# ebu/libear

Measured on AMD Instinct MI355X. Metric: Msamples/s, higher is better.
Workload: dtype f32 io / f16x2-split MFMA, f32 accumulate

## Files before the change

### libear_amd/csrc/api_core.hip

```cpp
#include <cctype>
#include <cerrno>
#include <cmath>
#include <cstdlib>
#include <string>
#include <memory>
#include <mutex>
#include <type_traits>

#include "common.h"
#include "curves.h"
#include "gain_kernels.h"
#include "gain_mfma.h"
#include "gain_h2.h"
#include "gain_h2_t1.h"
#include "gain_p2.h"
#include "gain_hg.h"
#include "gain_f32g.h"

namespace earhip {

static_assert(kSplitTile == 256, "MixLaunch::tile() and tiles_aligned(256, ...) assume the 4-wave tile");

static thread_local std::string g_last_error;
void set_last_error(const std::string &msg) { g_last_error = msg; }
// ... 363 lines not shown
    case GainKernel::Grid: launch_grid(c); break;
    case GainKernel::Pieces: launch_pieces(c); break;
    case GainKernel::Hinge:
      launch_hinge(c);
      if (c.standby) launch_pieces(c);
      break;
  }
  if (ev) EARHIP_HIP(hipEventRecord(ev[3], ctx->stream));
  EARHIP_HIP(hipGetLastError());
  MixResult res;
  res.gated = kind == GainKernel::Hinge && c.w.gate;
  res.device_form = c.w.wide_cur != nullptr;
  res.hinge_robust = res.gated && c.hg_robust;
  res.grew = c.w.grew;
  return res;
}

size_t hinge_build_allow_lds(const hipDeviceProp_t &prop) {
  const size_t want = 128 * 1024, dflt = 64 * 1024;
  const size_t device_max = std::max((size_t)prop.sharedMemPerBlock, (size_t)prop.maxSharedMemoryPerMultiProcessor);
  size_t ask = std::min(want, device_max > 4096 ? device_max - 4096 : dflt);
  if (ask <= dflt) return dflt;
  bool ok = true;
  for_each_hinge_build([&](auto T, auto NW) {
    ok = ok && hipFuncSetAttribute(reinterpret_cast<const void *>(&k_hinge_build<decltype(T)::value, decltype(NW)::value>),
                                   hipFuncAttributeMaxDynamicSharedMemorySize, (int)ask) == hipSuccess;
  });
  if (!ok) (void)hipGetLastError();
  return ok ? ask : dflt;
}

struct GainStage {
  earhip_ctx *ctx;
  int n_in, n_out;
  CurveSet curves;
  DevBuf<SegDesc> desc;
  DevBuf<float> parts;
  std::vector<float> rows;
  bool force_ramp;
  GainStage(earhip_ctx *c, int ni, int no, bool ramp = false)
      : ctx(c), n_in(ni), n_out(no), curves(ni, no, 1, ramp), force_ramp(ramp) {}

  void run_device(int64_t t_call, int nsamples, const float *in_dev, size_t in_stride,
                  float *out_dev, size_t out_stride) {
    curves.commit(ctx);
    const bool strict = ctx->strict || n_in == 1 || force_ramp;
    const MixLaunch ml = plan_mix(ctx, curves.plan(), n_in, nsamples, strict, 32, curves.stats(t_call, in_stride, (size_t)nsamples, false));
    if (ml.kind == GainKernel::Hinge) curves.ensure_kinks(ctx);
    desc.reserve(scratch_units(curves, ml, n_in));
    const size_t row_stride = ((size_t)nsamples + 3) & ~(size_t)3;
    if (ml.gsplit > 1) parts.reserve(row_stride * n_out * ml.gsplit);
    launch_gain_mix_summed(ctx, curves, ml, strict, t_call, nsamples, in_dev, in_stride, out_dev, out_stride, parts.p, row_stride, desc.p,
                           nullptr, nullptr);
  }

  void run_host(int64_t t_call, const float *const *in, float *const *out, int64_t r0,
                int64_t r1) {
    const int n = (int)(r1 - r0);
    if (n <= 0) return;
    const size_t stride = ((size_t)n + 3) & ~(size_t)3;
    ctx->pin_in.reserve(stride * n_in);
    ctx->pin_out.reserve(stride * n_out);
    ctx->dev_in.reserve(stride * n_in);
    ctx->dev_out.reserve(stride * n_out);
    for (int c = 0; c < n_in; c++)
      std::memcpy(ctx->pin_in.p + c * stride, in[c] + r0, sizeof(float) * n);
    EARHIP_HIP(hipMemcpyAsync(ctx->dev_in.p, ctx->pin_in.p, sizeof(float) * stride * n_in,
                              hipMemcpyHostToDevice, ctx->stream));
    run_device(t_call, n, ctx->dev_in.p, stride, ctx->dev_out.p, stride);
    EARHIP_HIP(hipMemcpyAsync(ctx->pin_out.p, ctx->dev_out.p, sizeof(float) * stride * n_out,
                              hipMemcpyDeviceToHost, ctx->stream));
    EARHIP_HIP(hipStreamSynchronize(ctx->stream));
    for (int c = 0; c < n_out; c++)
      std::memcpy(out[c] + r0, ctx->pin_out.p + c * stride, sizeof(float) * n);
  }
};

}

using namespace earhip;

static const char *const kOptNames[OPT_COUNT] = {
    "SPL", "MFMA", "XSCALE", "WAVES", "TPW", "NRT", "H2_TILE", "H2_WGS", "H2_RUNS", "P2_TILE", "P2_PAIRS", "P2_WGS", "HINGE", "HG_TILE", "HBUILD_TPW",
    "BUILD_TPW", "K2_WG", "K2_OWN_BLOCK", "RUN", "GSPLIT", "PROBE_RUNS", "BLOCK_GROUPS", "DEBUG_TIMING", "TAILCUT", "HOST_CHUNK_MB", "HOST_THREADS", "HG_ROBUST", "BUILD_2K", "HOST_BIND", "HOST_NT", "HOST_FIRST", "H2_PAIR"};

static int parse_option_value(const std::string &key, const char *text) {
  char *end = nullptr;
  errno = 0;
  const long v = std::strtol(text, &end, 10);
  while (end && *end && std::isspace((unsigned char)*end)) end++;
  if (end == text || (end && *end) || errno == ERANGE || v < -(1L << 30) || v > (1L << 30))
    fail_invalid("option '" + key + "': '" + std::string(text) + "' is not an integer");
  return (int)v;
}

void earhip_ctx::apply_options() {
  spl = 4, use_mfma = 3, x_scale_log2 = 14, x_scale_auto = true, max_waves = 4, tiles_per_wg = 4, tiles_per_wg_forced = false, nrt = 8;
  if (has(OPT_SPL) && (get(OPT_SPL) == 2 || get(OPT_SPL) == 4)) spl = get(OPT_SPL);
  if (has(OPT_MFMA)) use_mfma = get(OPT_MFMA);
  if (has(OPT_XSCALE) && get(OPT_XSCALE) >= -64 && get(OPT_XSCALE) <= 64)
    x_scale_log2 = get(OPT_XSCALE), x_scale_auto = false;
  if (has(OPT_WAVES) && get(OPT_WAVES) >= 1 && get(OPT_WAVES) <= 8) max_waves = get(OPT_WAVES);
  if (has(OPT_TPW) && get(OPT_TPW) >= 1 && get(OPT_TPW) <= 8) tiles_per_wg = get(OPT_TPW), tiles_per_wg_forced = true;
  if (has(OPT_NRT) && (get(OPT_NRT) == 4 || get(OPT_NRT) == 8)) nrt = get(OPT_NRT);
}

struct earhip_gain_interp {
  std::unique_ptr<GainStage> stage;
};

struct PolicyCache {
  std::vector<std::unique_ptr<GainStage>> stages;
  GainStage *get(earhip_ctx *ctx, int n_in, int n_out, bool ramp) {
    for (auto &s : stages)
      if (s->n_in == n_in && s->n_out == n_out && s->force_ramp == ramp) return s.get();
    stages.emplace_back(new GainStage(ctx, n_in, n_out, ramp));
    return stages.back().get();
  }
};
static std::vector<std::pair<earhip_ctx *, std::unique_ptr<PolicyCache>>> g_policy;
static std::mutex g_policy_mutex;
static PolicyCache *policy_cache(earhip_ctx *ctx) {
  std::lock_guard<std::mutex> lock(g_policy_mutex);
  for (auto &p : g_policy)
    if (p.first == ctx) return p.second.get();
  g_policy.emplace_back(ctx, std::unique_ptr<PolicyCache>(new PolicyCache));
  return g_policy.back().second.get();
}

static __global__ void k_clock_probe(unsigned long long *out) {
  out[0] = clock64();
  out[1] = wall_clock64();
}

static __global__ void __launch_bounds__(256) k_read_linear(const f32x4 *in, float *out, size_t n4) {
  f32x4 acc = {0.0f, 0.0f, 0.0f, 0.0f};
  size_t i = (size_t)blockIdx.x * 256 + threadIdx.x;
  const size_t step = (size_t)gridDim.x * 256;
  for (; i + 3 * step < n4; i += 4 * step) {
    const f32x4 a = __builtin_nontemporal_load(in + i), b = __builtin_nontemporal_load(in + i + step);
    const f32x4 c = __builtin_nontemporal_load(in + i + 2 * step), d = __builtin_nontemporal_load(in + i + 3 * step);
    acc += (a + b) + (c + d);
  }
  for (; i < n4; i += step) acc += __builtin_nontemporal_load(in + i);
  if (acc[0] + acc[1] + acc[2] + acc[3] == 123.456f) out[0] = 1.0f;
}
static __global__ void __launch_bounds__(256) k_read_rows(const float *in, float *out, int rows, size_t stride) {
  constexpr int DEPTH = 4;
  const int lane = threadIdx.x & 63, w = threadIdx.x >> 6, li = lane & 15, kg = lane >> 4;
  const float *base = in + (size_t)blockIdx.x * 256 + w * 64 + li * 4;
  auto row = [&](int r) { return base + (size_t)min(r, rows - 1) * stride; };
  f32x4 acc = {0.0f, 0.0f, 0.0f, 0.0f};
  f32x4 ring[DEPTH][8];
#pragma unroll
  for (int d = 0; d < DEPTH; d++)
#pragma unroll
    for (int q = 0; q < 8; q++)
      ring[d][q] = __builtin_nontemporal_load((const f32x4 *)row(d * 32 + kg * 8 + q));
  for (int r0 = 0; r0 < rows; r0 += 32 * DEPTH) {
#pragma unroll
    for (int d = 0; d < DEPTH; d++) {
#pragma unroll
      for (int q = 0; q < 8; q++) acc += ring[d][q];
      const int rn = r0 + 32 * DEPTH + d * 32;
      if (rn < rows)
#pragma unroll
        for (int q = 0; q < 8; q++)
// ... 406 lines not shown
```

### libear_amd/csrc/common.h

```cpp
#pragma once

#include <hip/hip_runtime.h>

#include <cstdint>
#include <cstdio>
#include <string>
#include <vector>

#include "../../include/earhip.h"

namespace earhip {

struct Error {
  int code;
  std::string msg;
};

void set_last_error(const std::string &msg);

template <typename F>
int guarded(F &&f) {
  try {
    f();
    return EARHIP_OK;
// ... 15 lines not shown
[[noreturn]] inline void fail_internal(const std::string &m) {
  throw Error{EARHIP_INTERNAL_ERROR, "internal error: " + m};
}
inline void require(bool ok, const char *m) {
  if (!ok) fail_invalid(m);
}

#define EARHIP_HIP(expr)                                                        \
  do {                                                                          \
    hipError_t e_ = (expr);                                                     \
    if (e_ != hipSuccess)                                                       \
      throw ::earhip::Error{EARHIP_DEVICE_ERROR,                                \
                            std::string("internal error: HIP: ") +              \
                                hipGetErrorString(e_) + " in " #expr};          \
  } while (0)

inline bool is_pow2(size_t v) { return v && !(v & (v - 1)); }

template <typename T>
struct DevBuf {
  T *p = nullptr;
  size_t n = 0;
  DevBuf() = default;
  DevBuf(const DevBuf &) = delete;
  DevBuf &operator=(const DevBuf &) = delete;
  ~DevBuf() { release(); }
  void release() {
    if (p) (void)hipFree(p);
    p = nullptr;
    n = 0;
  }
  void alloc(size_t count) {
    release();
    if (count == 0) count = 1;
    EARHIP_HIP(hipMalloc((void **)&p, count * sizeof(T)));
    n = count;
  }
  void alloc_zero(size_t count, hipStream_t s) {
    alloc(count);
    EARHIP_HIP(hipMemsetAsync(p, 0, n * sizeof(T), s));
  }
  void reserve(size_t count) {
    if (count > n) alloc(count);
  }
  void upload(const std::vector<T> &v) {
    alloc(v.size());
    if (!v.empty()) EARHIP_HIP(hipMemcpy(p, v.data(), sizeof(T) * v.size(), hipMemcpyHostToDevice));
  }
};

template <typename T>
struct PinBuf {
  T *p = nullptr;
  size_t n = 0;
  PinBuf() = default;
  PinBuf(const PinBuf &) = delete;
  PinBuf &operator=(const PinBuf &) = delete;
  ~PinBuf() {
    if (p) (void)hipHostFree(p);
  }
  void reserve(size_t count) {
    if (count <= n) return;
    if (p) (void)hipHostFree(p);
    p = nullptr;
    n = 0;
    EARHIP_HIP(hipHostMalloc((void **)&p, count * sizeof(T), hipHostMallocDefault));
    n = count;
  }
};

}

struct earhip_vbs;
namespace earhip {
void vbs_orphan(earhip_vbs *v);
}

namespace earhip {
enum Opt {
  OPT_SPL, OPT_MFMA, OPT_XSCALE, OPT_WAVES, OPT_TPW, OPT_NRT,
  OPT_H2_TILE, OPT_H2_WGS, OPT_H2_RUNS, OPT_P2_TILE, OPT_P2_PAIRS, OPT_P2_WGS, OPT_HINGE, OPT_HG_TILE, OPT_HBUILD_TPW, OPT_BUILD_TPW,
  OPT_K2_WG, OPT_K2_OWN_BLOCK, OPT_RUN, OPT_GSPLIT,
  OPT_PROBE_RUNS, OPT_BLOCK_GROUPS, OPT_DEBUG_TIMING, OPT_TAILCUT, OPT_HOST_CHUNK_MB, OPT_HOST_THREADS, OPT_HG_ROBUST, OPT_BUILD_2K,
  OPT_HOST_BIND, OPT_HOST_NT, OPT_HOST_FIRST, OPT_H2_PAIR, OPT_COUNT
};
struct OptVal {
  bool set = false;
  int v = 0;
};
}

struct earhip_ctx {
  earhip::OptVal opt[earhip::OPT_COUNT];
  bool has(earhip::Opt o) const { return opt[o].set; }
  int get(earhip::Opt o, int dflt = 0) const { return opt[o].set ? opt[o].v : dflt; }
  void apply_options();
  int device = 0;
  hipStream_t stream = nullptr;
  bool own_stream = false;
  bool strict = false;
  int spl = 4;
  int use_mfma = 3;
  int x_scale_log2 = 14;
  bool x_scale_auto = true;
  earhip::DevBuf<unsigned> level;
  int level_idx = 0;
  earhip::DevBuf<unsigned> tile_slow;
  size_t tile_slow_cap = 0;
  int tile_slow_idx = 0;
  earhip::DevBuf<unsigned> obj_level;
  int obj_level_cap = 0;
  long lazy_allocs = 0;
  int max_waves = 4;
  int tiles_per_wg = 4;
  bool tiles_per_wg_forced = false;
  int nrt = 8;
  int num_cus = 256;
  size_t hinge_build_lds = 64 * 1024;
  struct HostRange {
    const char *base;
    size_t bytes;
    bool owned;
  };
  std::vector<HostRange> host_ranges;
  std::vector<earhip_vbs *> pinned_adapters;
  bool host_reachable(const void *p, size_t bytes) const {
    const char *c = static_cast<const char *>(p);
    for (const auto &r : host_ranges)
      if (c >= r.base && c + bytes <= r.base + r.bytes) return true;
    return false;
  }
  earhip::PinBuf<float> pin_in, pin_out;
  earhip::DevBuf<float> dev_in, dev_out, dev_pts;
  void use() const { EARHIP_HIP(hipSetDevice(device)); }
};

namespace earhip {
int panner_create(earhip_ctx *ctx, const char *layout, int n_channels, const double *azimuth, const double *elevation,
                  earhip_panner **out, bool with_extent);
struct PanParams;
const PanParams &panner_params(const earhip_panner *p);
std::vector<double> panner_pan_points(earhip_panner *p, size_t npos, const double *xyz, unsigned *missed);
std::vector<double> tdesign_directions(size_t extra_rows = 0);
}
```

### libear_amd/csrc/decor_plan.h

```cpp
#pragma once

namespace earhip {

struct DecorPlan {
  int Bk = 0, Lk = 0;
  int NP = 1;
  int run_len = 11;
  bool run_len_set = false;
};

inline DecorPlan decor_plan(int K, int B, int n_taps, bool own_block, bool run_given, int run) {
  DecorPlan p;
  p.Bk = B;
  if (K == 2 && B > 512 && B % 512 == 0 && n_taps <= 512 && !own_block) p.Bk = 512;
  p.Lk = 2 * p.Bk;
  p.NP = (n_taps + p.Bk - 1) / p.Bk;
  if (p.Lk == 2048) p.run_len = 7;
  if (run_given && run >= 1 && run <= 255) p.run_len = run | 1, p.run_len_set = true;
  return p;
}

inline bool decor_wave_kernel(const DecorPlan &p, bool k2_wg) { return p.Lk == 1024 && p.NP == 1 && !k2_wg; }

inline int wave_run_len(int T, int N, int num_cus, int waves) {
  const double c[4] = {0.0, 6.9, 9.3, 12.2};
  int best = 1;
  double best_cost = 1e30;
  for (int R = 1; R <= 31; R += 2) {
    const long runs = (T + R - 1) / R;
    const long wgs = (runs + waves - 1) / waves * N;
    const long full = wgs / (3L * num_cus), rem = wgs - full * 3L * num_cus;
    const double pairs = (R + 1) / 2;
    const double cost = pairs * (full * c[3] + c[(rem + num_cus - 1) / num_cus]);
    if (cost <= best_cost) best_cost = cost, best = R;
    if (runs == 1) break;
  }
  return best;
}

}
```

### libear_amd/csrc/decor_stage.h

```cpp
#pragma once
#include <algorithm>

#include "common.h"
#include "decor_plan.h"
#include "fft_kernels.h"
#include "fft_launch.h"
#include "render_kernels.h"

namespace earhip {

static bool decor_fixed_size(int L) {
  bool fixed = false;
  fft_size_switch<128>(L, [&](auto) { fixed = true; }, [] {});
  return fixed;
}

static void launch_decor(int L, const DecorParams &P, dim3 grid, hipStream_t s) {
  fft_size_switch<128>(
      L, [&](auto LL) { hipLaunchKernelGGL((k_decorrelate_delay_mix<decltype(LL)::value>), grid, dim3(256), 0, s, P); },
      [&] {
        const FftShape S = shape_of(L, "block_size must be in [16, 4096]");
        const size_t lds = fft_rt_lds(k_decorrelate_delay_mix_rt, L, sizeof(float) * (L / 2));
        hipLaunchKernelGGL(k_decorrelate_delay_mix_rt, grid, dim3(256), lds, s, P, S);
      });
  EARHIP_HIP(hipGetLastError());
}

struct DecorStage : DecorPlan {
  int N = 0, B = 0, D = 0;
  DevBuf<cf> H, tw;
  DevBuf<float> tail[2], dly[2], hist[2];
  DevBuf<float> ztail, zdly, zhist;
  bool fresh = true;
  int cur = 0;
  int last_form = 0, last_R = 0;

  void create(earhip_ctx *ctx, const earhip_render_config &cfg, int block) {
    static_cast<DecorPlan &>(*this) =
        decor_plan(cfg.n_buses, block, cfg.n_taps, ctx->get(OPT_K2_OWN_BLOCK) != 0, ctx->has(OPT_RUN), ctx->get(OPT_RUN));
    N = cfg.n_out, B = block, D = cfg.delay;
    upload_twiddles(tw, Lk);
    const size_t rows = (size_t)NP * N;
    std::vector<float> parts(rows * Bk, 0.0f);
    for (int n = 0; n < N; n++)
      for (int t = 0; t < cfg.n_taps; t++)
        parts[((size_t)(t / Bk) * N + n) * Bk + t % Bk] = cfg.decorrelators[(size_t)n * cfg.n_taps + t];
    DevBuf<float> taps;
    taps.alloc(parts.size());
    EARHIP_HIP(hipMemcpy(taps.p, parts.data(), sizeof(float) * parts.size(), hipMemcpyHostToDevice));
    H.alloc(rows * Lk);
    launch_spectrum(Lk, taps.p, Bk, Bk, tw.p, H.p, (int)rows, ctx->stream);
    EARHIP_HIP(hipStreamSynchronize(ctx->stream));
    std::vector<cf> h(rows * Lk);
    EARHIP_HIP(hipMemcpy(h.data(), H.p, sizeof(cf) * h.size(), hipMemcpyDeviceToHost));
    for (size_t n = 0; n < rows; n++) {
      cf *hn = h.data() + n * Lk;
      hn[0].y = 0.0f;
      hn[Bk].y = 0.0f;
      for (int k = 1; k < Bk; k++) hn[Lk - k] = cf_conj(hn[k]);
    }
    EARHIP_HIP(hipMemcpy(H.p, h.data(), sizeof(cf) * h.size(), hipMemcpyHostToDevice));
    const size_t hist_n = (size_t)N * std::max((NP - 1) * Bk, 1);
    for (int i = 0; i < 2; i++) {
      tail[i].alloc_zero(rows * Bk, ctx->stream);
      dly[i].alloc_zero((size_t)N * std::max(D, 1), ctx->stream);
      hist[i].alloc_zero(hist_n, ctx->stream);
      if (i == 0) {
        ztail.alloc_zero((size_t)N * Bk, ctx->stream);
        zdly.alloc_zero((size_t)N * std::max(D, 1), ctx->stream);
        zhist.alloc_zero(hist_n, ctx->stream);
      }
    }
  }

  void reset() { fresh = true; }

  void run(earhip_ctx *ctx, size_t nblocks, int nsamples, float *bus, size_t bus_stride, size_t part_stride, int nparts, float *out,
           size_t out_stride, hipEvent_t *evp) {
    DecorParams P;
    P.bus = bus;
    P.bus_stride = bus_stride;
    P.part_stride = part_stride;
    P.nparts = nparts;
    const bool wave_k2 = decor_wave_kernel(*this, ctx->get(OPT_K2_WG) != 0);
    const int kblocks = (int)(nblocks * (size_t)(B / Bk));
    if (wave_k2 && nparts > 1) {
      if (evp) EARHIP_HIP(hipEventRecord(evp[4], ctx->stream));
      hipLaunchKernelGGL(k_sum_parts, dim3((nsamples + 255) / 256, 2 * N), dim3(256), 0, ctx->stream, bus, part_stride, nparts,
                         bus_stride, 2 * N, nsamples, bus, bus_stride);
      EARHIP_HIP(hipGetLastError());
      P.nparts = 1;
    }
    P.out = out;
    P.out_stride = out_stride;
    P.tw = tw.p;
    P.dly_in = fresh ? zdly.p : dly[cur].p;
    P.dly_out = dly[cur ^ 1].p;
    P.N = N;
    P.T = kblocks;
    const int R = wave_k2 && !run_len_set ? wave_run_len(kblocks, N, ctx->num_cus, kDecorWaves) : run_len;
    P.R = R;
    last_form = wave_k2 ? 2 : decor_fixed_size(Lk) ? 0 : 1;
    last_R = R;
    P.D = D;
    P.hist_len = (NP - 1) * Bk;
    P.hist_in = fresh ? zhist.p : hist[cur].p;
    P.hist_out = hist[cur ^ 1].p;
    const dim3 grid((unsigned)((kblocks + R - 1) / R), N);
    if (evp && P.nparts == nparts) EARHIP_HIP(hipEventRecord(evp[4], ctx->stream));
    for (int part = 0; part < NP; part++) {
      P.H = H.p + (size_t)part * N * Lk;
      P.tail_in = (fresh ? ztail.p : tail[cur].p) + (fresh ? 0 : (size_t)part * N * Bk);
      P.tail_out = tail[cur ^ 1].p + (size_t)part * N * Bk;
      P.shift = part * Bk;
      P.accumulate = part > 0 ? 1 : 0;
      if (wave_k2) {
        hipLaunchKernelGGL(k_decorrelate_wave, dim3((grid.x + kDecorWaves - 1) / kDecorWaves, grid.y), dim3(64 * kDecorWaves),
                           0, ctx->stream, P);
        EARHIP_HIP(hipGetLastError());
      } else {
        launch_decor(Lk, P, grid, ctx->stream);
      }
    }
    if (evp) EARHIP_HIP(hipEventRecord(evp[5], ctx->stream));
    cur ^= 1;
    fresh = false;
  }
};

}
```

### libear_amd/csrc/render_kernels.h

```cpp
#pragma once

#include <hip/hip_runtime.h>

#include "fft_lds.h"

namespace earhip {

struct DecorParams {
  const float *bus;
  size_t bus_stride;
  size_t part_stride;
  int nparts;
  float *out;
  size_t out_stride;
  const cf *H;
  const cf *tw;
  const float *tail_in;
  float *tail_out;
  const float *dly_in;
  float *dly_out;
  int N, T, R, D;
  int shift = 0;
  int accumulate = 0;
  int hist_len = 0;
  const float *hist_in = nullptr;
  float *hist_out = nullptr;
};

template <int DIR>
__device__ __forceinline__ void r4_core_w(cf v0, cf v1, cf v2, cf v3, cf *out, int Ns, int j,
                                          const cf (&w)[3]) {
  const int k = j & (Ns - 1);
  v1 = cf_mul(v1, DIR > 0 ? cf_conj(w[0]) : w[0]);
  v2 = cf_mul(v2, DIR > 0 ? cf_conj(w[1]) : w[1]);
  v3 = cf_mul(v3, DIR > 0 ? cf_conj(w[2]) : w[2]);
  const cf a0 = cf_add(v0, v2), a1 = cf_sub(v0, v2);
  const cf a2 = cf_add(v1, v3), a3 = cf_mul_i<DIR>(cf_sub(v1, v3));
  const int base = ((j - k) << 2) + k;
  out[base] = cf_add(a0, a2);
  out[base + Ns] = cf_add(a1, a3);
  out[base + 2 * Ns] = cf_sub(a0, a2);
  out[base + 3 * Ns] = cf_sub(a1, a3);
}

template <int DIR>
__device__ __forceinline__ void r4_vals_w(cf v0, cf v1, cf v2, cf v3, const cf (&w)[3], cf (&o)[4]) {
  v1 = cf_mul(v1, DIR > 0 ? cf_conj(w[0]) : w[0]);
  v2 = cf_mul(v2, DIR > 0 ? cf_conj(w[1]) : w[1]);
  v3 = cf_mul(v3, DIR > 0 ? cf_conj(w[2]) : w[2]);
  const cf a0 = cf_add(v0, v2), a1 = cf_sub(v0, v2);
  const cf a2 = cf_add(v1, v3), a3 = cf_mul_i<DIR>(cf_sub(v1, v3));
  o[0] = cf_add(a0, a2);
  o[1] = cf_add(a1, a3);
  o[2] = cf_sub(a0, a2);
  o[3] = cf_sub(a1, a3);
}

template <int L, int DIR, int NT>
__device__ __forceinline__ cf *fft_run_passes_w(cf *src, cf *dst, const cf (&twr)[fft_r4_passes(L) - 1][3],
                                                int first, int stop, int tid) {
  constexpr int NR4 = fft_r4_passes(L);
  static_assert(!fft_has_r2(L) && L / 4 == NT, "power-of-four length, one butterfly per thread");
  int Ns = 1;
  for (int p = 0; p < first; ++p) Ns *= 4;
#pragma unroll
  for (int p = 0; p < NR4; ++p) {
    if (p < first || p >= stop) continue;
    __syncthreads();
    if (p == 0) stockham_r4<L, DIR>(src, dst, nullptr, 1, tid);
    else r4_core_w<DIR>(src[tid], src[tid + L / 4], src[tid + L / 2], src[tid + 3 * L / 4], dst, Ns, tid, twr[p - 1]);
    cf *t = src;
    src = dst;
    dst = t;
    Ns *= 4;
  }
  return src;
}

template <int L, int DIR, int NT>
__device__ __forceinline__ cf *fft_r4_range(cf *src, cf *dst, const cf *tw, int first, int stop, int tid) {
  int Ns = 1;
  for (int p = 0; p < first; ++p) Ns *= 4;
#pragma unroll
  for (int p = 0; p < fft_r4_passes(L); ++p) {
    if (p < first || p >= stop) continue;
    __syncthreads();
// ... 712 lines not shown
    }
#ifdef EARHIP_K2_PROF
    asm volatile("" : "+v"(v[0]));
    EARHIP_K2_MARK(prof_i + 3);
#endif
    wave_fft1024<+1>(v, lds, t1, t2, lane);
#ifdef EARHIP_K2_PROF
    asm volatile("" : "+v"(v[0]));
    EARHIP_K2_MARK(prof_i + 4);
    prof_i += 5;
#endif
#pragma unroll
    for (int m = 0; m < 8; m++) {
      dre[m] = (v[m].x + tl[m]) * norm + dre[m];
      asm volatile("" : "+v"(dre[m]) : : "memory");
      tl[m] = have_re ? v[m + 8].x : tl[m];
    }
#pragma unroll
    for (int m = 0; m < 8; m++) {
      dim[m] = (v[m].y + tl[m]) * norm + dim[m];
      asm volatile("" : "+v"(dim[m]) : : "memory");
      tl[m] = have_im ? v[m + 8].y : tl[m];
    }
#pragma unroll
    for (int m = 0; m < 8; m++) {
      v[m] = z[m];
      asm volatile("" : "+v"(v[m]) : : "memory");
    }
    __builtin_amdgcn_sched_barrier(0);
#if EARHIP_K2_ABL == 1 || EARHIP_K2_ABL == 3
    if (have_im && dre[0] + dim[0] + dre[7] + dim[7] == 123.456f) out[tb * B + lane] = dre[1] + dim[1];
#else
    if (have_re && tb >= first) {
#pragma unroll
      for (int m = 0; m < 8; m++) __builtin_nontemporal_store(dre[m], out + tb * B + lane + 64 * m);
    }
    if (have_im) {
#pragma unroll
      for (int m = 0; m < 8; m++) __builtin_nontemporal_store(dim[m], out + (tb + 1) * B + lane + 64 * m);
    }
#endif
  }
  EARHIP_K2_MARK(prof_i < 31 ? prof_i : 31);
  if (last == P.T) {
#pragma unroll
    for (int m = 0; m < 8; m++) P.tail_out[(size_t)n * B + lane + 64 * m] = tl[m];
    const int total = P.T * B;
    if (total >= P.D && P.D <= 256) {
      const float *q = direct + (total - P.D) + lane;
      float acc[4] = {0.0f, 0.0f, 0.0f, 0.0f};
      bool ok[4];
#pragma unroll
      for (int k = 0; k < 4; k++) ok[k] = lane + 64 * k < P.D;
      int p = 0;
      for (; p + 3 < P.nparts; p += 4) {
        float t[4][4];
#pragma unroll
        for (int j = 0; j < 4; j++)
#pragma unroll
          for (int k = 0; k < 4; k++) t[j][k] = ok[k] ? q[(size_t)(p + j) * P.part_stride + 64 * k] : 0.0f;
#pragma unroll
        for (int k = 0; k < 4; k++) {
          acc[k] = p == 0 ? t[0][k] : acc[k] + t[0][k];
          acc[k] += t[1][k];
          acc[k] += t[2][k];
          acc[k] += t[3][k];
        }
      }
      for (; p < P.nparts; p++)
#pragma unroll
        for (int k = 0; k < 4; k++) {
          const float v = ok[k] ? q[(size_t)p * P.part_stride + 64 * k] : 0.0f;
          acc[k] = p == 0 ? v : acc[k] + v;
        }
#pragma unroll
      for (int k = 0; k < 4; k++)
        if (ok[k]) P.dly_out[(size_t)n * P.D + lane + 64 * k] = acc[k];
    } else {
      for (int j = lane; j < P.D; j += 64) P.dly_out[(size_t)n * P.D + j] = delayed(total + j);
    }
  }
}


}
```

Baseline: 1.148 million.

## Add even-odd paired decorrelation kernel packing two real blocks per complex FFT

Adds a new decorrelation kernel for the 1024-point single-partition case. It packs two consecutive real input blocks into the real and imaginary halves of one complex FFT, so each overlap-save step runs half as many FFT round trips. Work is split into pair runs per wave by a new planner. Because the kernel carries the previous raw input block instead of the convolution tail, a small conversion kernel is added to rebuild the tail when a later call falls back to the old path. The packed form is chosen by default whenever the wave path is eligible and the run length is above one. It adds state-handoff complexity and relies on the two packed outputs staying separable.

```diff
diff --git a/libear_amd/csrc/api_core.hip b/libear_amd/csrc/api_core.hip
--- a/libear_amd/csrc/api_core.hip
+++ b/libear_amd/csrc/api_core.hip
@@ -469,7 +469,8 @@
 
 static const char *const kOptNames[OPT_COUNT] = {
     "SPL", "MFMA", "XSCALE", "WAVES", "TPW", "NRT", "H2_TILE", "H2_WGS", "H2_RUNS", "P2_TILE", "P2_PAIRS", "P2_WGS", "HINGE", "HG_TILE", "HBUILD_TPW",
-    "BUILD_TPW", "K2_WG", "K2_OWN_BLOCK", "RUN", "GSPLIT", "PROBE_RUNS", "BLOCK_GROUPS", "DEBUG_TIMING", "TAILCUT", "HOST_CHUNK_MB", "HOST_THREADS", "HG_ROBUST", "BUILD_2K", "HOST_BIND", "HOST_NT", "HOST_FIRST", "H2_PAIR"};
+    "BUILD_TPW", "K2_WG", "K2_OWN_BLOCK", "RUN", "GSPLIT", "PROBE_RUNS", "BLOCK_GROUPS", "DEBUG_TIMING", "TAILCUT", "HOST_CHUNK_MB", "HOST_THREADS", "HG_ROBUST", "BUILD_2K", "HOST_BIND", "HOST_NT", "HOST_FIRST", "H2_PAIR",
+    "K2_EVEN", "K2_EVEN_PAIRS"};
 
 static int parse_option_value(const std::string &key, const char *text) {
   char *end = nullptr;
diff --git a/libear_amd/csrc/common.h b/libear_amd/csrc/common.h
--- a/libear_amd/csrc/common.h
+++ b/libear_amd/csrc/common.h
@@ -121,7 +121,9 @@
   OPT_H2_TILE, OPT_H2_WGS, OPT_H2_RUNS, OPT_P2_TILE, OPT_P2_PAIRS, OPT_P2_WGS, OPT_HINGE, OPT_HG_TILE, OPT_HBUILD_TPW, OPT_BUILD_TPW,
   OPT_K2_WG, OPT_K2_OWN_BLOCK, OPT_RUN, OPT_GSPLIT,
   OPT_PROBE_RUNS, OPT_BLOCK_GROUPS, OPT_DEBUG_TIMING, OPT_TAILCUT, OPT_HOST_CHUNK_MB, OPT_HOST_THREADS, OPT_HG_ROBUST, OPT_BUILD_2K,
-  OPT_HOST_BIND, OPT_HOST_NT, OPT_HOST_FIRST, OPT_H2_PAIR, OPT_COUNT
+  OPT_HOST_BIND, OPT_HOST_NT, OPT_HOST_FIRST, OPT_H2_PAIR,
+  OPT_K2_EVEN, OPT_K2_EVEN_PAIRS,
+  OPT_COUNT
 };
 struct OptVal {
   bool set = false;
diff --git a/libear_amd/csrc/decor_plan.h b/libear_amd/csrc/decor_plan.h
--- a/libear_amd/csrc/decor_plan.h
+++ b/libear_amd/csrc/decor_plan.h
@@ -38,4 +38,24 @@
   return best;
 }
 
+struct DecorEvenPlan {
+  int waves = 0;
+  int pairs = 0;
+};
+inline DecorEvenPlan decor_even_plan(int T, int N, int num_cus, int fixed_pairs = 0) {
+  const int total = T > 1 ? (T + 1) / 2 : 1;
+  int wc = 12 * num_cus / N;
+  wc = wc < 1 ? 1 : wc > total ? total : wc;
+  DecorEvenPlan p;
+  p.pairs = fixed_pairs > 0 ? fixed_pairs : (total + wc - 1) / wc;
+  p.waves = (total + p.pairs - 1) / p.pairs;
+  return p;
 }
+
+inline bool decor_even_form(bool wave_eligible, bool even_set, int even_opt, bool run_len_set, int R) {
+  if (!wave_eligible) return false;
+  if (even_set) return even_opt != 0;
+  return !run_len_set && R > 1;
+}
+
+}
diff --git a/libear_amd/csrc/decor_stage.h b/libear_amd/csrc/decor_stage.h
--- a/libear_amd/csrc/decor_stage.h
+++ b/libear_amd/csrc/decor_stage.h
@@ -30,6 +30,8 @@
   int N = 0, B = 0, D = 0;
   DevBuf<cf> H, tw;
   DevBuf<float> tail[2], dly[2], hist[2];
+  DevBuf<float> last[2];
+  bool state_block = false;
   DevBuf<float> ztail, zdly, zhist;
   bool fresh = true;
   int cur = 0;
@@ -65,6 +67,7 @@
       tail[i].alloc_zero(rows * Bk, ctx->stream);
       dly[i].alloc_zero((size_t)N * std::max(D, 1), ctx->stream);
       hist[i].alloc_zero(hist_n, ctx->stream);
+      if (Lk == 1024 && NP == 1) last[i].alloc_zero((size_t)N * Bk, ctx->stream);
       if (i == 0) {
         ztail.alloc_zero((size_t)N * Bk, ctx->stream);
         zdly.alloc_zero((size_t)N * std::max(D, 1), ctx->stream);
@@ -84,8 +87,13 @@
     P.nparts = nparts;
     const bool wave_k2 = decor_wave_kernel(*this, ctx->get(OPT_K2_WG) != 0);
     const int kblocks = (int)(nblocks * (size_t)(B / Bk));
+    bool stamped = false;
+    auto stamp = [&] {
+      if (evp && !stamped) EARHIP_HIP(hipEventRecord(evp[4], ctx->stream));
+      stamped = true;
+    };
     if (wave_k2 && nparts > 1) {
-      if (evp) EARHIP_HIP(hipEventRecord(evp[4], ctx->stream));
+      stamp();
       hipLaunchKernelGGL(k_sum_parts, dim3((nsamples + 255) / 256, 2 * N), dim3(256), 0, ctx->stream, bus, part_stride, nparts,
                          bus_stride, 2 * N, nsamples, bus, bus_stride);
       EARHIP_HIP(hipGetLastError());
@@ -100,15 +108,40 @@
     P.T = kblocks;
     const int R = wave_k2 && !run_len_set ? wave_run_len(kblocks, N, ctx->num_cus, kDecorWaves) : run_len;
     P.R = R;
-    last_form = wave_k2 ? 2 : decor_fixed_size(Lk) ? 0 : 1;
+    const bool even = decor_even_form(wave_k2, ctx->has(OPT_K2_EVEN), ctx->get(OPT_K2_EVEN), run_len_set, R);
+    last_form = even ? 3 : wave_k2 ? 2 : decor_fixed_size(Lk) ? 0 : 1;
     last_R = R;
     P.D = D;
     P.hist_len = (NP - 1) * Bk;
     P.hist_in = fresh ? zhist.p : hist[cur].p;
     P.hist_out = hist[cur ^ 1].p;
     const dim3 grid((unsigned)((kblocks + R - 1) / R), N);
-    if (evp && P.nparts == nparts) EARHIP_HIP(hipEventRecord(evp[4], ctx->stream));
-    for (int part = 0; part < NP; part++) {
+    stamp();
+    if (even) {
+      const DecorEvenPlan ep = decor_even_plan(kblocks, N, ctx->num_cus, std::min(ctx->get(OPT_K2_EVEN_PAIRS), 1 << 20));
+      DecorEvenParams E{};
+      static_cast<DecorParams &>(E) = P;
+      E.H = H.p;
+      E.tail_in = fresh || state_block ? nullptr : tail[cur].p;
+      E.last_in = fresh || !state_block ? nullptr : last[cur].p;
+      E.last_out = last[cur ^ 1].p;
+      E.pairs = ep.pairs;
+      last_R = 2 * ep.pairs;
+      hipLaunchKernelGGL(k_decorrelate_even<false>, dim3((ep.waves + kDecorWaves - 1) / kDecorWaves, N), dim3(64 * kDecorWaves), 0,
+                         ctx->stream, E);
+      EARHIP_HIP(hipGetLastError());
+    } else if (!fresh && state_block) {
+      DecorEvenParams E{};
+      E.H = H.p;
+      E.tw = tw.p;
+      E.last_in = last[cur].p;
+      E.tail_out = tail[cur].p;
+      E.N = N, E.T = 1;
+      hipLaunchKernelGGL(k_decorrelate_even<true>, dim3(1, N), dim3(64 * kDecorWaves), 0, ctx->stream, E);
+      EARHIP_HIP(hipGetLastError());
+    }
+    state_block = even;
+    for (int part = 0; part < NP && !even; part++) {
       P.H = H.p + (size_t)part * N * Lk;
       P.tail_in = (fresh ? ztail.p : tail[cur].p) + (fresh ? 0 : (size_t)part * N * Bk);
       P.tail_out = tail[cur ^ 1].p + (size_t)part * N * Bk;
diff --git a/libear_amd/csrc/render_kernels.h b/libear_amd/csrc/render_kernels.h
--- a/libear_amd/csrc/render_kernels.h
+++ b/libear_amd/csrc/render_kernels.h
@@ -880,5 +880,162 @@
   }
 }
 
-
-}
+struct DecorEvenParams : DecorParams {
+  const float *last_in = nullptr;
+  float *last_out = nullptr;
+  int pairs = 1;
+};
+
+template <bool CONVERT>
+__global__ void __launch_bounds__(64 * kDecorWaves) __attribute__((amdgpu_waves_per_eu(3, 3))) k_decorrelate_even(DecorEvenParams P) {
+  constexpr int L = 1024, B = 512;
+  __shared__ v2f lds_all[kDecorWaves][L + L / 16];
+  __shared__ v2f h_lds[L + L / 16];
+  __shared__ v2f t1_lds[16][17];
+  __shared__ v2f t2_lds[3 * 256];
+  const int lane = threadIdx.x & 63, w = __builtin_amdgcn_readfirstlane(threadIdx.x >> 6);
+  v2f *lds = lds_all[w];
+  auto to_v2f = [](cf c) { return v2f{c.x, c.y}; };
+  const int n = blockIdx.y;
+  for (int i = threadIdx.x; i < L; i += 64 * kDecorWaves) h_lds[wave_pad(i)] = to_v2f(P.H[(size_t)n * L + i]);
+  if (threadIdx.x < 240) {
+    const int k = threadIdx.x / 15, r = threadIdx.x % 15 + 1;
+    t1_lds[k][r - 1] = to_v2f(P.tw[(4 * r * k) & (L - 1)]);
+  }
+  for (int i = threadIdx.x; i < 3 * 256; i += 64 * kDecorWaves) t2_lds[i] = to_v2f(P.tw[((i >> 8) + 1) * (i & 255)]);
+  __syncthreads();
+  const int first = (blockIdx.x * kDecorWaves + w) * 2 * P.pairs;
+  if (first >= P.T) return;
+  const int last = min(first + 2 * P.pairs, P.T);
+  const v2f *t1 = t1_lds[lane & 15];
+  const v2f *t2 = t2_lds;
+  v2f v[16];
+
+  if (CONVERT) {
+#pragma unroll
+    for (int m = 0; m < 8; m++) {
+      v[m] = v2f{P.last_in[(size_t)n * B + lane + 64 * m], 0.0f};
+      v[m + 8] = v2f{0.0f, 0.0f};
+    }
+    wave_fft1024<-1, true>(v, lds, t1, t2, lane);
+#pragma unroll
+    for (int m = 0; m < 16; m++) v[m] = wave_cmul<-1>(v[m], h_lds[wave_pad(lane + 64 * m)]);
+    wave_fft1024<+1>(v, lds, t1, t2, lane);
+#pragma unroll
+    for (int m = 0; m < 8; m++) P.tail_out[(size_t)n * B + lane + 64 * m] = v[m + 8].x;
+    return;
+  }
+
+  const float norm = 1.0f / (float)(2 * B);
+  const float *direct = P.bus + (size_t)n * P.bus_stride;
+  const float *diffuse = P.bus + (size_t)(P.N + n) * P.bus_stride;
+  float *out = P.out + (size_t)n * P.out_stride;
+
+  auto delayed = [&](int s) {
+    const int sd = s - P.D;
+    return sd >= 0 ? direct[sd] : P.dly_in[(size_t)n * P.D + (sd + P.D)];
+  };
+  auto delayed8 = [&](int tb, float (&acc)[8]) {
+    const int s0 = tb * B - P.D + lane;
+    const float *q = direct + s0;
+    if (tb * B >= P.D) {
+#pragma unroll
+      for (int m = 0; m < 8; m++) acc[m] = __builtin_nontemporal_load(q + 64 * m);
+    } else {
+#pragma unroll
+      for (int m = 0; m < 8; m++)
+        acc[m] = s0 + 64 * m < 0 ? P.dly_in[(size_t)n * P.D + (s0 + 64 * m + P.D)] : q[64 * m];
+    }
+  };
+  auto load_block = [&](int tb, v2f (&z)[8], auto im_tag) {
+    constexpr bool IM = decltype(im_tag)::value;
+    const float *q = diffuse + tb * B + lane;
+#pragma unroll
+    for (int m = 0; m < 8; m++) {
+      const float x = __builtin_nontemporal_load(q + 64 * m);
+      if (IM) z[m].y = x;
+      else z[m].x = x;
+    }
+  };
+  auto load_pair = [&](int tb, v2f (&z)[8]) {
+#pragma unroll
+    for (int m = 0; m < 8; m++) z[m] = v2f{0.0f, 0.0f};
+    if (tb < last) load_block(tb, z, std::false_type{});
+    if (tb + 1 < last) load_block(tb + 1, z, std::true_type{});
+  };
+
+  float tl[8];
+  float c[8];
+#pragma unroll
+  for (int m = 0; m < 8; m++) {
+    tl[m] = first == 0 && P.tail_in ? P.tail_in[(size_t)n * B + lane + 64 * m] : 0.0f;
+    c[m] = 0.0f;
+    if (first > 0) c[m] = __builtin_nontemporal_load(diffuse + (first - 1) * B + lane + 64 * m);
+    else if (P.last_in) c[m] = P.last_in[(size_t)n * B + lane + 64 * m];
+  }
+  {
+    v2f z[8];
+    load_pair(first, z);
+#pragma unroll
+    for (int m = 0; m < 8; m++) v[m] = v2f{c[m], z[m].x}, v[m + 8] = z[m];
+  }
+  for (int tb = first; tb < last; tb += 2) {
+    const bool have_im = tb + 1 < last;
+#pragma unroll
+    for (int m = 0; m < 8; m++) c[m] = have_im ? v[m + 8].y : v[m].y;
+    v2f z[8];
+    load_pair(tb + 2, z);
+    float dre[8], dim[8];
+#pragma unroll
+    for (int m = 0; m < 8; m++) dim[m] = 0.0f;
+    delayed8(tb, dre);
+    if (have_im) delayed8(tb + 1, dim);
+    wave_fft1024<-1, false>(v, lds, t1, t2, lane);
+#pragma unroll
+    for (int m = 0; m < 16; m++) {
+      v[m] = wave_cmul<-1>(v[m], h_lds[wave_pad(lane + 64 * m)]);
+      if ((m & 3) == 3) __builtin_amdgcn_sched_barrier(0);
+    }
+    wave_fft1024<+1>(v, lds, t1, t2, lane);
+#pragma unroll
+    for (int m = 0; m < 8; m++) {
+      dre[m] = (v[m + 8].x + tl[m]) * norm + dre[m];
+      asm volatile("" : "+v"(dre[m]) : : "memory");
+      tl[m] = 0.0f;
+    }
+#pragma unroll
+    for (int m = 0; m < 8; m++) {
+      dim[m] = v[m + 8].y * norm + dim[m];
+      asm volatile("" : "+v"(dim[m]) : : "memory");
+    }
+#pragma unroll
+    for (int m = 0; m < 8; m++) {
+      v[m] = v2f{c[m], z[m].x};
+      v[m + 8] = z[m];
+      asm volatile("" : "+v"(v[m]), "+v"(v[m + 8]) : : "memory");
+    }
+    __builtin_amdgcn_sched_barrier(0);
+#pragma unroll
+    for (int m = 0; m < 8; m++) __builtin_nontemporal_store(dre[m], out + tb * B + lane + 64 * m);
+    if (have_im) {
+#pragma unroll
+      for (int m = 0; m < 8; m++) __builtin_nontemporal_store(dim[m], out + (tb + 1) * B + lane + 64 * m);
+    }
+  }
+  if (last == P.T) {
+#pragma unroll
+    for (int m = 0; m < 8; m++) P.last_out[(size_t)n * B + lane + 64 * m] = c[m];
+    const int total = P.T * B;
+    if (total >= P.D && P.D <= 256) {
+      const float *q = direct + (total - P.D) + lane;
+#pragma unroll
+      for (int k = 0; k < 4; k++)
+        if (lane + 64 * k < P.D) P.dly_out[(size_t)n * P.D + lane + 64 * k] = q[64 * k];
+    } else {
+      for (int j = lane; j < P.D; j += 64) P.dly_out[(size_t)n * P.D + j] = delayed(total + j);
+    }
+  }
+}
+
+
+}
```

New measurement: 1.127 million. 0.982x the previous value.

## Add even-split decorrelation kernel packing two real blocks per complex FFT

Applied to the files above, without the earlier changes.

Adds a new decorrelation kernel that splits block pairs evenly across waves and packs two consecutive real overlap-save blocks into the real and imaginary halves of one complex 1024-point FFT. This roughly halves the FFT work per block and balances load across CUs. Cross-call state is carried as the raw last input block rather than a convolved tail. A small conversion kernel rebuilds the tail when falling back to the old path. The new path is chosen automatically when there is enough work, adding complexity in state handling and edge cases for odd block counts.

```diff
diff --git a/libear_amd/csrc/api_core.hip b/libear_amd/csrc/api_core.hip
--- a/libear_amd/csrc/api_core.hip
+++ b/libear_amd/csrc/api_core.hip
@@ -469,7 +469,7 @@
 
 static const char *const kOptNames[OPT_COUNT] = {
     "SPL", "MFMA", "XSCALE", "WAVES", "TPW", "NRT", "H2_TILE", "H2_WGS", "H2_RUNS", "P2_TILE", "P2_PAIRS", "P2_WGS", "HINGE", "HG_TILE", "HBUILD_TPW",
-    "BUILD_TPW", "K2_WG", "K2_OWN_BLOCK", "RUN", "GSPLIT", "PROBE_RUNS", "BLOCK_GROUPS", "DEBUG_TIMING", "TAILCUT", "HOST_CHUNK_MB", "HOST_THREADS", "HG_ROBUST", "BUILD_2K", "HOST_BIND", "HOST_NT", "HOST_FIRST", "H2_PAIR"};
+    "BUILD_TPW", "K2_WG", "K2_OWN_BLOCK", "RUN", "GSPLIT", "PROBE_RUNS", "BLOCK_GROUPS", "DEBUG_TIMING", "TAILCUT", "HOST_CHUNK_MB", "HOST_THREADS", "HG_ROBUST", "BUILD_2K", "HOST_BIND", "HOST_NT", "HOST_FIRST", "H2_PAIR", "K2_EVEN"};
 
 static int parse_option_value(const std::string &key, const char *text) {
   char *end = nullptr;
diff --git a/libear_amd/csrc/common.h b/libear_amd/csrc/common.h
--- a/libear_amd/csrc/common.h
+++ b/libear_amd/csrc/common.h
@@ -121,7 +121,9 @@
   OPT_H2_TILE, OPT_H2_WGS, OPT_H2_RUNS, OPT_P2_TILE, OPT_P2_PAIRS, OPT_P2_WGS, OPT_HINGE, OPT_HG_TILE, OPT_HBUILD_TPW, OPT_BUILD_TPW,
   OPT_K2_WG, OPT_K2_OWN_BLOCK, OPT_RUN, OPT_GSPLIT,
   OPT_PROBE_RUNS, OPT_BLOCK_GROUPS, OPT_DEBUG_TIMING, OPT_TAILCUT, OPT_HOST_CHUNK_MB, OPT_HOST_THREADS, OPT_HG_ROBUST, OPT_BUILD_2K,
-  OPT_HOST_BIND, OPT_HOST_NT, OPT_HOST_FIRST, OPT_H2_PAIR, OPT_COUNT
+  OPT_HOST_BIND, OPT_HOST_NT, OPT_HOST_FIRST, OPT_H2_PAIR,
+  OPT_K2_EVEN,
+  OPT_COUNT
 };
 struct OptVal {
   bool set = false;
diff --git a/libear_amd/csrc/decor_plan.h b/libear_amd/csrc/decor_plan.h
--- a/libear_amd/csrc/decor_plan.h
+++ b/libear_amd/csrc/decor_plan.h
@@ -38,4 +38,36 @@
   return best;
 }
 
+#if defined(__HIPCC__)
+#define EARHIP_PLAN_FN __host__ __device__ inline
+#else
+#define EARHIP_PLAN_FN inline
+#endif
+
+struct EvenPlan {
+  bool take = false;
+  int W = 0;
+  int P = 0;
+};
+
+EARHIP_PLAN_FN int even_pair_begin(int P, int W, int i) { return (int)((long long)P * i / W); }
+
+inline EvenPlan even_plan(int T, int N, int num_cus) {
+  EvenPlan e;
+  e.W = 4 * (3 * num_cus / N);
+  e.P = (T + 1) / 2;
+  e.take = T >= 2 && e.W >= 4 && (long)e.P * N >= 2L * 12 * num_cus;
+  return e;
 }
+
+inline int even_max_blocks(int T, const EvenPlan &e) {
+  int most = 0;
+  for (int i = 0; i < e.W; i++) {
+    const int j0 = even_pair_begin(e.P, e.W, i), j1 = even_pair_begin(e.P, e.W, i + 1);
+    const int blocks = 2 * (j1 - j0) - ((j1 == e.P && j1 > j0 && (T & 1)) ? 1 : 0);
+    if (blocks > most) most = blocks;
+  }
+  return most;
+}
+
+}
diff --git a/libear_amd/csrc/decor_stage.h b/libear_amd/csrc/decor_stage.h
--- a/libear_amd/csrc/decor_stage.h
+++ b/libear_amd/csrc/decor_stage.h
@@ -30,6 +30,8 @@
   int N = 0, B = 0, D = 0;
   DevBuf<cf> H, tw;
   DevBuf<float> tail[2], dly[2], hist[2];
+  DevBuf<float> last[2];
+  bool state_last = false;
   DevBuf<float> ztail, zdly, zhist;
   bool fresh = true;
   int cur = 0;
@@ -63,6 +65,7 @@
     const size_t hist_n = (size_t)N * std::max((NP - 1) * Bk, 1);
     for (int i = 0; i < 2; i++) {
       tail[i].alloc_zero(rows * Bk, ctx->stream);
+      last[i].alloc_zero((size_t)N * Bk, ctx->stream);
       dly[i].alloc_zero((size_t)N * std::max(D, 1), ctx->stream);
       hist[i].alloc_zero(hist_n, ctx->stream);
       if (i == 0) {
@@ -84,8 +87,43 @@
     P.nparts = nparts;
     const bool wave_k2 = decor_wave_kernel(*this, ctx->get(OPT_K2_WG) != 0);
     const int kblocks = (int)(nblocks * (size_t)(B / Bk));
+    bool started = false;
+    auto start = [&] {
+      if (evp && !started) EARHIP_HIP(hipEventRecord(evp[4], ctx->stream));
+      started = true;
+    };
+    const EvenPlan ev = even_plan(kblocks, N, ctx->num_cus);
+    const bool even_ok = wave_k2 && !run_len_set && !ctx->has(OPT_RUN) && nparts == 1 && kblocks >= 2 && ev.W >= 4;
+    if (even_ok && (ctx->has(OPT_K2_EVEN) ? ctx->get(OPT_K2_EVEN) != 0 : ev.take)) {
+      DecorEvenParams E;
+      E.bus = bus, E.bus_stride = bus_stride;
+      E.out = out, E.out_stride = out_stride;
+      E.H = H.p, E.tw = tw.p;
+      E.prev_in = fresh ? ztail.p : state_last ? last[cur].p : tail[cur].p;
+      E.prev_is_tail = !fresh && !state_last ? 1 : 0;
+      E.last_out = last[cur ^ 1].p;
+      E.dly_in = fresh ? zdly.p : dly[cur].p;
+      E.dly_out = dly[cur ^ 1].p;
+      E.N = N, E.T = kblocks, E.D = D;
+      start();
+      hipLaunchKernelGGL(k_decorrelate_even, dim3(ev.W / kDecorWaves, N), dim3(64 * kDecorWaves), 0, ctx->stream, E);
+      EARHIP_HIP(hipGetLastError());
+      if (evp) EARHIP_HIP(hipEventRecord(evp[5], ctx->stream));
+      last_form = 3;
+      last_R = even_max_blocks(kblocks, ev);
+      cur ^= 1;
+      fresh = false;
+      state_last = true;
+      return;
+    }
+    if (!fresh && state_last) {
+      start();
+      hipLaunchKernelGGL(k_decor_last_to_tail, dim3(N), dim3(64), 0, ctx->stream, last[cur].p, H.p, tw.p, tail[cur].p);
+      EARHIP_HIP(hipGetLastError());
+    }
+    state_last = false;
     if (wave_k2 && nparts > 1) {
-      if (evp) EARHIP_HIP(hipEventRecord(evp[4], ctx->stream));
+      start();
       hipLaunchKernelGGL(k_sum_parts, dim3((nsamples + 255) / 256, 2 * N), dim3(256), 0, ctx->stream, bus, part_stride, nparts,
                          bus_stride, 2 * N, nsamples, bus, bus_stride);
       EARHIP_HIP(hipGetLastError());
@@ -107,7 +145,7 @@
     P.hist_in = fresh ? zhist.p : hist[cur].p;
     P.hist_out = hist[cur ^ 1].p;
     const dim3 grid((unsigned)((kblocks + R - 1) / R), N);
-    if (evp && P.nparts == nparts) EARHIP_HIP(hipEventRecord(evp[4], ctx->stream));
+    start();
     for (int part = 0; part < NP; part++) {
       P.H = H.p + (size_t)part * N * Lk;
       P.tail_in = (fresh ? ztail.p : tail[cur].p) + (fresh ? 0 : (size_t)part * N * Bk);
diff --git a/libear_amd/csrc/render_kernels.h b/libear_amd/csrc/render_kernels.h
--- a/libear_amd/csrc/render_kernels.h
+++ b/libear_amd/csrc/render_kernels.h
@@ -2,6 +2,7 @@
 
 #include <hip/hip_runtime.h>
 
+#include "decor_plan.h"
 #include "fft_lds.h"
 
 namespace earhip {
@@ -880,5 +881,178 @@
   }
 }
 
-
-}
+struct DecorEvenParams {
+  const float *bus;
+  size_t bus_stride;
+  float *out;
+  size_t out_stride;
+  const cf *H;
+  const cf *tw;
+  const float *prev_in;
+  int prev_is_tail;
+  float *last_out;
+  const float *dly_in;
+  float *dly_out;
+  int N, T, D;
+};
+
+__global__ void __launch_bounds__(64 * kDecorWaves) __attribute__((amdgpu_waves_per_eu(3, 3))) k_decorrelate_even(DecorEvenParams P) {
+  constexpr int L = 1024, B = 512;
+  __shared__ v2f lds_all[kDecorWaves][L + L / 16];
+  __shared__ v2f h_lds[L + L / 16];
+  __shared__ v2f t1_lds[16][17];
+  __shared__ v2f t2_lds[3 * 256];
+  const int lane = threadIdx.x & 63, w = __builtin_amdgcn_readfirstlane(threadIdx.x >> 6);
+  v2f *lds = lds_all[w];
+  auto to_v2f = [](cf c) { return v2f{c.x, c.y}; };
+  const int n = blockIdx.y;
+  for (int i = threadIdx.x; i < L; i += 64 * kDecorWaves) h_lds[wave_pad(i)] = to_v2f(P.H[(size_t)n * L + i]);
+  if (threadIdx.x < 240) {
+    const int k = threadIdx.x / 15, r = threadIdx.x % 15 + 1;
+    t1_lds[k][r - 1] = to_v2f(P.tw[(4 * r * k) & (L - 1)]);
+  }
+  for (int i = threadIdx.x; i < 3 * 256; i += 64 * kDecorWaves) t2_lds[i] = to_v2f(P.tw[((i >> 8) + 1) * (i & 255)]);
+  __syncthreads();
+  const int pairs = (P.T + 1) >> 1, waves = (int)gridDim.x * kDecorWaves, gw = (int)blockIdx.x * kDecorWaves + w;
+  const int j0 = even_pair_begin(pairs, waves, gw), j1 = even_pair_begin(pairs, waves, gw + 1);
+  if (j0 >= j1) return;
+  const float norm = 1.0f / (float)(2 * B);
+  const float *direct = P.bus + (size_t)n * P.bus_stride;
+  const float *diffuse = P.bus + (size_t)(P.N + n) * P.bus_stride;
+  float *out = P.out + (size_t)n * P.out_stride;
+  const v2f *t1 = t1_lds[lane & 15];
+  const v2f *t2 = t2_lds;
+
+  auto delayed = [&](int s) {
+    const int sd = s - P.D;
+    return sd >= 0 ? direct[sd] : P.dly_in[(size_t)n * P.D + (sd + P.D)];
+  };
+  auto delayed8 = [&](int tb, float (&acc)[8]) {
+    const int s0 = tb * B - P.D + lane;
+    const float *q = direct + s0;
+    if (tb * B >= P.D) {
+#pragma unroll
+      for (int m = 0; m < 8; m++) acc[m] = __builtin_nontemporal_load(q + 64 * m);
+    } else {
+#pragma unroll
+      for (int m = 0; m < 8; m++) acc[m] = s0 + 64 * m < 0 ? P.dly_in[(size_t)n * P.D + (s0 + 64 * m + P.D)] : q[64 * m];
+    }
+  };
+  auto load_pair = [&](int j, v2f (&z)[8]) {
+#pragma unroll
+    for (int m = 0; m < 8; m++) z[m] = v2f{0.0f, 0.0f};
+    if (j >= j1) return;
+    const float *q = diffuse + (size_t)(2 * j) * B + lane;
+#pragma unroll
+    for (int m = 0; m < 8; m++) z[m].x = __builtin_nontemporal_load(q + 64 * m);
+    if (2 * j + 1 < P.T) {
+#pragma unroll
+      for (int m = 0; m < 8; m++) z[m].y = __builtin_nontemporal_load(q + B + 64 * m);
+    }
+  };
+
+  v2f v[16];
+  {
+    float a[8];
+#pragma unroll
+    for (int m = 0; m < 8; m++) a[m] = 0.0f;
+    if (j0 > 0) {
+#pragma unroll
+      for (int m = 0; m < 8; m++) a[m] = diffuse[(size_t)(2 * j0 - 1) * B + lane + 64 * m];
+    } else if (!P.prev_is_tail) {
+#pragma unroll
+      for (int m = 0; m < 8; m++) a[m] = P.prev_in[(size_t)n * B + lane + 64 * m];
+    }
+    v2f z[8];
+    load_pair(j0, z);
+#pragma unroll
+    for (int m = 0; m < 8; m++) v[m] = v2f{a[m], z[m].x}, v[m + 8] = z[m];
+  }
+  float keep[8];
+  for (int j = j0; j < j1; j++) {
+    const bool have_im = 2 * j + 1 < P.T;
+#pragma unroll
+    for (int m = 0; m < 8; m++) keep[m] = have_im ? v[m + 8].y : v[m + 8].x;
+    v2f z[8];
+    load_pair(j + 1, z);
+    float dre[8], dim[8];
+#pragma unroll
+    for (int m = 0; m < 8; m++) dim[m] = 0.0f;
+    delayed8(2 * j, dre);
+    if (have_im) delayed8(2 * j + 1, dim);
+    if (j == 0 && P.prev_is_tail) {
+#pragma unroll
+      for (int m = 0; m < 8; m++) dre[m] += P.prev_in[(size_t)n * B + lane + 64 * m] * norm;
+    }
+    wave_fft1024<-1>(v, lds, t1, t2, lane);
+#pragma unroll
+    for (int m = 0; m < 16; m++) {
+      v[m] = wave_cmul<-1>(v[m], h_lds[wave_pad(lane + 64 * m)]);
+      if ((m & 3) == 3) __builtin_amdgcn_sched_barrier(0);
+    }
+    wave_fft1024<+1>(v, lds, t1, t2, lane);
+#pragma unroll
+    for (int m = 0; m < 8; m++) {
+      dre[m] = v[m + 8].x * norm + dre[m];
+      asm volatile("" : "+v"(dre[m]) : : "memory");
+    }
+#pragma unroll
+    for (int m = 0; m < 8; m++) {
+      dim[m] = v[m + 8].y * norm + dim[m];
+      asm volatile("" : "+v"(dim[m]) : : "memory");
+    }
+#pragma unroll
+    for (int m = 0; m < 8; m++) {
+      v[m] = v2f{keep[m], z[m].x};
+      v[m + 8] = z[m];
+      asm volatile("" : "+v"(v[m]), "+v"(v[m + 8]) : : "memory");
+    }
+    __builtin_amdgcn_sched_barrier(0);
+#pragma unroll
+    for (int m = 0; m < 8; m++) __builtin_nontemporal_store(dre[m], out + (size_t)(2 * j) * B + lane + 64 * m);
+    if (have_im) {
+#pragma unroll
+      for (int m = 0; m < 8; m++) __builtin_nontemporal_store(dim[m], out + (size_t)(2 * j + 1) * B + lane + 64 * m);
+    }
+  }
+  if (j1 == pairs) {
+#pragma unroll
+    for (int m = 0; m < 8; m++) P.last_out[(size_t)n * B + lane + 64 * m] = keep[m];
+    const int total = P.T * B;
+    if (total >= P.D && P.D <= 256) {
+      const float *q = direct + (total - P.D) + lane;
+#pragma unroll
+      for (int k = 0; k < 4; k++)
+        if (lane + 64 * k < P.D) P.dly_out[(size_t)n * P.D + lane + 64 * k] = q[64 * k];
+    } else {
+      for (int i = lane; i < P.D; i += 64) P.dly_out[(size_t)n * P.D + i] = delayed(total + i);
+    }
+  }
+}
+
+__global__ void __launch_bounds__(64) k_decor_last_to_tail(const float *last, const cf *H, const cf *tw, float *tail) {
+  constexpr int L = 1024, B = 512;
+  __shared__ v2f lds[L + L / 16];
+  __shared__ v2f t1_lds[16][17];
+  __shared__ v2f t2_lds[3 * 256];
+  const int lane = threadIdx.x, n = blockIdx.x;
+  auto to_v2f = [](cf c) { return v2f{c.x, c.y}; };
+  for (int i = lane; i < 240; i += 64) {
+    const int k = i / 15, r = i % 15 + 1;
+    t1_lds[k][r - 1] = to_v2f(tw[(4 * r * k) & (L - 1)]);
+  }
+  for (int i = lane; i < 3 * 256; i += 64) t2_lds[i] = to_v2f(tw[((i >> 8) + 1) * (i & 255)]);
+  __syncthreads();
+  v2f v[16];
+#pragma unroll
+  for (int m = 0; m < 8; m++) v[m] = v2f{last[(size_t)n * B + lane + 64 * m], 0.0f}, v[m + 8] = v2f{0.0f, 0.0f};
+  wave_fft1024<-1, true>(v, lds, t1_lds[lane & 15], t2_lds, lane);
+#pragma unroll
+  for (int m = 0; m < 16; m++) v[m] = wave_cmul<-1>(v[m], to_v2f(H[(size_t)n * L + lane + 64 * m]));
+  wave_fft1024<+1>(v, lds, t1_lds[lane & 15], t2_lds, lane);
+#pragma unroll
+  for (int m = 0; m < 8; m++) tail[(size_t)n * B + lane + 64 * m] = v[m + 8].x;
+}
+
+
+}
```

After: 1.165 million before, 1.179 million after (median of 6 runs). 1.01x the previous value.
